# AssafSinger94/dino-tracker

Measured on AMD Instinct MI355X. Metric: query-points*frames/s, higher is better.
Workload: dtype mixed: fp16 ViT operands (one per value), f16 conv operands in Delta-DINO, f16 candidates + f32 deciders in the tracker; f32 accumulate; 1 GPU; 854x480x90 synthetic video (model res 854x476, 67x121 tokens, C=384), 1024 grid queries; 1 video(s) per step over 1 GPU(s); features=vit, mode=single, track_method=mfma, anchor_pairs=92091, correlation_maps_per_video=8380350, rccl_ranks=1, parallelism=video-parallel x1

## Files before the change

dino_tracker_amd/csrc/vit.hip:

```cpp
#include <stdlib.h>
#include "common.h"
#include "vit_attention4.h"
#include "vit_attention6.h"
#include "vit_gemm_common.h"
#include "vit_gemm_tiled.h"
#include "vit_gemm_ws.h"
#include "vit_gemm_wide.h"
#include "vit_split.h"

namespace {

__global__ __launch_bounds__(256) void patch_embed_kernel(const float* __restrict__ frames, const float* __restrict__ Wp,
                                                          const float* __restrict__ bp, const float* __restrict__ pos,
                                                          const float* __restrict__ cls_pos,
                                                          const float* __restrict__ mean_std, float* __restrict__ x,
                                                          int H, int W, int ph, int pw, int D, int patch, int stride,
                                                          int S) {
    const int HW = ph * pw;
    const int K = 3 * patch * patch;
    const int frame = blockIdx.z;
    const int tid = threadIdx.x, lane = tid & 63, w = tid >> 6;
    const int p0 = blockIdx.x * 64 + (w >> 1) * 32;
    const int n0 = blockIdx.y * 64 + (w & 1) * 32;
    const int li = lane & 31, lk = lane >> 5;
// ... 262 lines not shown
VitPlan vit_plan(const dtk_vit_model* m, int ph, int pw, int frames) {
    VitPlan p;
    p.S = ph * pw + 1;
    p.Sp = (p.S + 127) / 128 * 128;
    const int fb = m->frame_batch > 0 ? m->frame_batch : VIT_FRAME_BATCH;
    p.FB = frames < fb ? frames : fb;
    auto al = [](size_t v) { return (v + 255) & ~(size_t)255; };
    size_t off = 0;
    const size_t rows = (size_t)p.FB * p.S;
    p.x = off; off = al(off + rows * m->D * 4);
    p.xn = off; off = al(off + rows * m->D * 2);
    p.q = off; off = al(off + (size_t)p.FB * m->heads * p.Sp * 64 * 2);
    p.k = off; off = al(off + (size_t)p.FB * m->heads * p.Sp * 64 * 2);
    p.vt = off; off = al(off + (size_t)p.FB * m->heads * p.Sp * 64 * 2);
    p.ao = off; off = al(off + rows * m->D * 2);
    p.hid = off; off = al(off + rows * 4 * m->D * 2);
    p.delta = off; off = al(off + rows * m->D * 2);
    p.split = false;
    for (int l = 0; l < m->depth; ++l) p.split |= vit_layer_split(m->layers[l]);
    p.xn_lo = p.q_lo = p.k_lo = p.vt_lo = p.ao_lo = p.hid_lo = 0;
    if (p.split) {
        p.xn_lo = off; off = al(off + rows * m->D * 2);
        p.q_lo = off; off = al(off + (size_t)p.FB * m->heads * p.Sp * 64 * 2);
        p.k_lo = off; off = al(off + (size_t)p.FB * m->heads * p.Sp * 64 * 2);
        p.vt_lo = off; off = al(off + (size_t)p.FB * m->heads * p.Sp * 64 * 2);
        p.ao_lo = off; off = al(off + rows * m->D * 2);
        p.hid_lo = off; off = al(off + rows * 4 * m->D * 2);
    }
    p.total = off;
    return p;
}

template <typename T>
int attention_launch(const T* q, const T* k, const T* vt, T* o, int S, int Sp, int heads, int D, int FH, bool v4, hipStream_t st) {
    int QB;
    if (v4) {
        const unsigned grid = attn::attention_grid(FH, S, 256, &QB);
        DTK_LAUNCH("vit_attention", (attn::attention4_kernel<T, 0>), dim3(grid), dim3(256), 0, st, q, k, vt, o, S, Sp, heads, D,
                   FH, QB);
    } else {
        const unsigned grid = attn::attention_grid(FH, S, 128 * attn::A6_NQ, &QB);
        DTK_LAUNCH("vit_attention", (attn::attention6_kernel<T, 0>), dim3(grid), dim3(256), 0, st, q, k, vt, o, S, Sp, heads, D,
                   FH, QB);
    }
    return DTK_OK;
}

template <typename T>
__global__ __launch_bounds__(256) void range_scan_kernel(const T* __restrict__ p, long long n8, int* __restrict__ flag, int bit) {
    typedef typename Vec<T>::t8 T8;
    bool bad = false;
    for (long long i = (long long)blockIdx.x * 256 + threadIdx.x; i < n8; i += (long long)gridDim.x * 256) {
        const T8 v = reinterpret_cast<const T8*>(p)[i];
#pragma unroll
        for (int e = 0; e < 8; ++e) bad |= !(fabsf((float)v[e]) < 65504.f);
    }
    if (__any(bad) && (threadIdx.x & 63) == 0) atomicOr(flag, bit);
}

struct GemmPath {
    bool tiled;
    bool ws;
    bool wide;
    bool ws_v1;
    bool wide_v1;
    bool fc2_ln;
};
inline GemmPath gemm_path(int D, int f) {
    const bool tiled = (f & DTK_VIT_TILED_GEMMS) != 0, ws = !tiled && D == WS_K, wide_v1 = (f & DTK_VIT_GEMM_WIDE_V1) != 0;
    static_assert(WS_K == WD_N, "fc2 of the weight-stationary width is gemm_wide_delta_kernel's shape");
    return {tiled, ws, !tiled && D % W2_N == 0, (f & DTK_VIT_GEMM_WS_V1) != 0, wide_v1, ws && !wide_v1 && !(f & DTK_VIT_NO_LN_FUSION)};
}
inline GemmPath gemm_path(const dtk_vit_model* m) { return gemm_path(m->D, m->flags); }

template <typename T, int EPI>
int launch_gemm(const char* name, const GemmPath& path, const T* A, const T* W, long long rows, int N, int K, const GemmEpi<T>& e,
                hipStream_t st) {
    if constexpr (EPI != EPI_F32) {
        const bool ws_fits = EPI != EPI_QKV || e.S >= WS_ROWS || rows <= e.S;
        if (path.ws && K == WS_K && ws_fits) {
            const auto gr = gemm_ws_grid(N, rows);
            if (path.ws_v1)
                DTK_LAUNCH(name, (gemm_ws_kernel<T, EPI, 0>), gr.first, dim3(256), 0, st, A, W, rows, N, e, gr.second);
            else
                DTK_LAUNCH(name, (gemm_ws_kernel<T, EPI>), gr.first, dim3(256), 0, st, A, W, rows, N, e, gr.second);
            return DTK_OK;
        }
        if (path.ws && EPI == EPI_DELTA) {
            const dim3 grid(dtk_cdiv(rows, WD_M));
            if (path.wide_v1)
                DTK_LAUNCH(name, (gemm_wide_delta_kernel<T, false>), grid, dim3(512), 0, st, A, W, rows, K, e);
            else if (e.ln_out)
                DTK_LAUNCH(name, (gemm_wide_delta_kernel<T, true, true>), grid, dim3(512), 0, st, A, W, rows, K, e);
            else
                DTK_LAUNCH(name, (gemm_wide_delta_kernel<T, true>), grid, dim3(512), 0, st, A, W, rows, K, e);
            return DTK_OK;
        }
        if (path.wide) {
            const dim3 grid(gemm_wide_grid(N, rows));
            if (path.wide_v1)
                DTK_LAUNCH(name, (gemm_wide_kernel<T, EPI, false>), grid, dim3(512), 0, st, A, W, rows, N, K, e);
            else
                DTK_LAUNCH(name, (gemm_wide_kernel<T, EPI, true>), grid, dim3(512), 0, st, A, W, rows, N, K, e);
            return DTK_OK;
        }
    }
    DTK_LAUNCH(name, (gemm_tiled_kernel<T, EPI>), dim3(gemm_grid(N, rows)), dim3(256), 0, st, A, W, rows, N, K, e);
    return DTK_OK;
}

template <typename T, int SEPI>
int launch_gemm_split(const char* name, const GemmPath& path, const T* Ah, const T* Al, const T* Wh, const T* Wl, long long rows,
                      int N, int K, const SplitEpi<T>& se, hipStream_t st) {
    if (!path.tiled && N % SD_N == 0) {
        const dim3 grid(gemm_split_dma_grid(N, rows));
        if (path.wide_v1)
            DTK_LAUNCH(name, (gemm_split_dma_kernel<T, SEPI, false>), grid, dim3(512), 0, st, Ah, Al, Wh, Wl, rows, N, K, se);
        else
            DTK_LAUNCH(name, (gemm_split_dma_kernel<T, SEPI, true>), grid, dim3(512), 0, st, Ah, Al, Wh, Wl, rows, N, K, se);
        return DTK_OK;
    }
    DTK_LAUNCH(name, (gemm_split_kernel<T, SEPI>), dim3(gemm_split_grid(N, rows)), dim3(256), 0, st, Ah, Al, Wh, Wl, rows, N, K, se);
    return DTK_OK;
}

template <typename T>
int vit_run(const dtk_vit_model* m, const float* frames, int nframes, int video_h, int video_w, float* tokens_out,
            float* feat_out, float* qkv_out, unsigned char* ws, const VitPlan& p, int ph, int pw, hipStream_t st) {
    const int HW = ph * pw, D = m->D;
    float* x = reinterpret_cast<float*>(ws + p.x);
    auto at = [&](size_t off) { return reinterpret_cast<T*>(ws + off); };
    T *xn = at(p.xn), *q = at(p.q), *k = at(p.k), *vt = at(p.vt), *ao = at(p.ao), *hid = at(p.hid), *delta = at(p.delta);
    T *xn_lo = at(p.xn_lo), *q_lo = at(p.q_lo), *k_lo = at(p.k_lo), *vt_lo = at(p.vt_lo), *ao_lo = at(p.ao_lo), *hid_lo = at(p.hid_lo);
    int* ovf = m->overflow;
    const bool scan_all = ovf && (m->flags & DTK_VIT_CHECK_RANGE);
    int* const epi_ovf = IsF16<T>::value ? ovf : nullptr;
    const int S = p.S, Sp = p.Sp;
    {
        const long long n16 = (long long)((p.ao - p.q) / 16);
        DTK_LAUNCH("vit_zero", zero_kernel, dim3(dtk_cdiv(n16, 256)), dim3(256), 0, st, reinterpret_cast<uint4*>(q), n16);
        if (p.split) {
            const long long m16 = (long long)((p.ao_lo - p.q_lo) / 16);
            DTK_LAUNCH("vit_zero", zero_kernel, dim3(dtk_cdiv(m16, 256)), dim3(256), 0, st, reinterpret_cast<uint4*>(q_lo), m16);
        }
    }
    for (int f0 = 0; f0 < nframes; f0 += p.FB) {
        const int nf = (nframes - f0) < p.FB ? (nframes - f0) : p.FB;
        const long long rows = (long long)nf * S;
        auto scan_range = [&](const T* t, long long n, int bit) -> int {
            const int blocks = (int)(dtk_cdiv(n / 8, 256) < 1024 ? dtk_cdiv(n / 8, 256) : 1024);
            DTK_LAUNCH("vit_range_scan", range_scan_kernel<T>, dim3(blocks), dim3(256), 0, st, t, n / 8, ovf, bit);
            return DTK_OK;
        };
        const bool pe_fits = (size_t)nf * video_h * video_w * 16 <= p.delta - p.hid &&
                             (size_t)D * PE_K * 4 <= p.total - p.delta;
        if (m->patch == PE_P && m->stride == PE_S && pe_fits) {
            h4v* fh = reinterpret_cast<h4v*>(hid);
            h4v* fl = fh + (size_t)nf * video_h * video_w;
            half_t* wh = reinterpret_cast<half_t*>(delta);
            half_t* wl = wh + (size_t)D * PE_K;
            const long long npix = (long long)nf * video_h * video_w;
            DTK_LAUNCH("vit_frame_split", frame_split4_kernel, dim3(dtk_cdiv(npix, 256)), dim3(256), 0, st,
                       frames + (size_t)f0 * 3 * video_h * video_w, m->mean_std, fh, fl, video_h, video_w, npix);
            DTK_LAUNCH("vit_frame_split", pack_patch_split_kernel, dim3(dtk_cdiv((long long)D * PE_K, 256)), dim3(256), 0, st,
                       m->patch_w, D, wh, wl);
            const int groups_x = dtk_cdiv(pw, PE_TOK);
            const int units = groups_x * ph * nf, slabs = dtk_cdiv(D, PE_NF);
            DTK_LAUNCH("vit_patch_embed", patch_embed_split_kernel, dim3(8 * dtk_cdiv(units, 8) * slabs), dim3(256), 0, st, fh,
                       fl, wh, wl, m->patch_b, m->pos, m->cls_pos, x, video_h, video_w, ph, pw, D, S, groups_x, units, slabs);
        } else {
            DTK_LAUNCH("vit_patch_embed", patch_embed_kernel, dim3(dtk_cdiv(HW, 64), dtk_cdiv(D, 64), nf), dim3(256), 0, st,
                       frames + (size_t)f0 * 3 * video_h * video_w, m->patch_w, m->patch_b, m->pos, m->cls_pos, m->mean_std,
                       x, video_h, video_w, ph, pw, D, m->patch, m->stride, S);
        }
        const GemmPath path = gemm_path(m);
        const int dbg_ns = DTK_DBG(dtk_dev_flags() >> 16, 0x7f);
        bool pending = false;
        bool ln1_done = false;
        auto tap = [&](int l, bool with_delta) -> int {
            if (!m->tap_out || !((m->tap_mask >> l) & 1)) return DTK_OK;
            const long long t4 = rows * (D / 4);
            DTK_LAUNCH("vit_tap", tap_kernel<T>, dim3(dtk_cdiv(t4, 256)), dim3(256), 0, st, x, with_delta ? (const T*)delta : (const T*)nullptr,
                       m->tap_out + (size_t)f0 * S * D, m->tap_scale, t4);
            return DTK_OK;
        };
        for (int l = 0; l < m->depth; ++l) {
            const dtk_vit_layer& L = m->layers[l];
            const T* qkv_w = reinterpret_cast<const T*>(L.qkv_w);
            const T* proj_w = reinterpret_cast<const T*>(L.proj_w);
            const T* fc1_w = reinterpret_cast<const T*>(L.fc1_w);
            const T* fc2_w = reinterpret_cast<const T*>(L.fc2_w);
            if (vit_layer_split(L)) {
                const T* qkv_wl = reinterpret_cast<const T*>(L.qkv_w_lo);
                const T* proj_wl = reinterpret_cast<const T*>(L.proj_w_lo);
                const T* fc1_wl = reinterpret_cast<const T*>(L.fc1_w_lo);
                const T* fc2_wl = reinterpret_cast<const T*>(L.fc2_w_lo);
                const float inv_ws = 1.f / (L.w_scale > 0.f ? L.w_scale : 1.f);
                DTK_LAUNCH("vit_layernorm_split", layernorm_split_kernel<T>, dim3(dtk_cdiv(rows, 4)), dim3(256), 0, st, x,
                           pending ? (const T*)delta : (const T*)nullptr, L.ln1_w, L.ln1_b, xn, xn_lo, rows, D, m->ln_eps, ovf);
                pending = false;
                SplitEpi<T> se{};
                if (qkv_out && l == m->depth - 1) {
                    se.bias = L.qkv_b; se.inv_wscale = inv_ws; se.out_f32 = qkv_out + (size_t)f0 * S * 3 * D;
                    if (launch_gemm_split<T, SEPI_F32>("vit_gemm_qkv_facet", path, xn, xn_lo, qkv_w, qkv_wl, rows, 3 * D, D, se, st)) return DTK_E_HIP;
                    se = SplitEpi<T>{};
                }
                se.bias = L.qkv_b; se.inv_wscale = inv_ws; se.q_hi = q; se.q_lo = q_lo; se.k_hi = k; se.k_lo = k_lo; se.vt_hi = vt;
                se.vt_lo = vt_lo; se.S = S; se.Sp = Sp; se.heads = m->heads; se.D = D; se.qscale = 0.125f * 1.4426950408889634f;
                se.ovf = epi_ovf;
                if (launch_gemm_split<T, SEPI_QKV>("vit_gemm_qkv_split", path, xn, xn_lo, qkv_w, qkv_wl, rows, 3 * D, D, se, st)) return DTK_E_HIP;
                const int nqb = dtk_cdiv(Sp, 128);
                DTK_LAUNCH("vit_attention_split", attention_split_kernel<T>, dim3((unsigned)(nf * m->heads * nqb)), dim3(256), 0, st,
                           (const T*)q, (const T*)q_lo, (const T*)k, (const T*)k_lo, (const T*)vt, (const T*)vt_lo, ao, ao_lo, S, Sp,
                           m->heads, nqb);
                se = SplitEpi<T>{};
                se.bias = L.proj_b; se.inv_wscale = inv_ws; se.x = x; se.gamma = L.ls1;
                if (launch_gemm_split<T, SEPI_RESID>("vit_gemm_proj_split", path, ao, ao_lo, proj_w, proj_wl, rows, D, D, se, st)) return DTK_E_HIP;
                DTK_LAUNCH("vit_layernorm_split", layernorm_split_kernel<T>, dim3(dtk_cdiv(rows, 4)), dim3(256), 0, st, x,
                           (const T*)nullptr, L.ln2_w, L.ln2_b, xn, xn_lo, rows, D, m->ln_eps, ovf);
                se = SplitEpi<T>{};
                se.bias = L.fc1_b; se.inv_wscale = inv_ws; se.out_hi = hid; se.out_lo = hid_lo; se.ovf = epi_ovf;
                if (launch_gemm_split<T, SEPI_GELU>("vit_gemm_fc1_split", path, xn, xn_lo, fc1_w, fc1_wl, rows, 4 * D, D, se, st)) return DTK_E_HIP;
                se = SplitEpi<T>{};
                se.bias = L.fc2_b; se.inv_wscale = inv_ws; se.x = x; se.gamma = L.ls2;
                if (launch_gemm_split<T, SEPI_RESID>("vit_gemm_fc2_split", path, hid, hid_lo, fc2_w, fc2_wl, rows, D, 4 * D, se, st)) return DTK_E_HIP;
                if (tap(l, false)) return DTK_E_HIP;
                continue;
            }
            GemmEpi<T> e{};
            if (!ln1_done)
                DTK_LAUNCH("vit_layernorm", layernorm_kernel<T>, dim3(dtk_cdiv(rows, 4)), dim3(256), 0, st, x,
                           pending ? (const T*)delta : (const T*)nullptr, L.ln1_w, L.ln1_b, xn, rows, D, m->ln_eps, ovf);
            ln1_done = false;
            pending = true;
            if (qkv_out && l == m->depth - 1) {
                e.bias = L.qkv_b; e.out_f32 = qkv_out + (size_t)f0 * S * 3 * D;
                if (launch_gemm<T, EPI_F32>("vit_gemm_qkv_facet", path, xn, qkv_w, rows, 3 * D, D, e, st)) return DTK_E_HIP;
                e = GemmEpi<T>{};
            }
            e.bias = L.qkv_b; e.q = q; e.k = k; e.vt = vt; e.S = S; e.Sp = Sp; e.heads = m->heads; e.D = D;
            e.qscale = 0.125f * 1.4426950408889634f; e.no_store = dbg_ns; e.ovf = epi_ovf;
            if (launch_gemm<T, EPI_QKV>("vit_gemm_qkv", path, xn, qkv_w, rows, 3 * D, D, e, st)) return DTK_E_HIP;
            if (scan_all && scan_range(q, (long long)(p.ao - p.q) / 2, 2)) return DTK_E_HIP;
            if (attention_launch(q, k, vt, ao, S, Sp, m->heads, D, nf * m->heads, (m->flags & DTK_VIT_ATTENTION_V4) != 0, st)) return DTK_E_HIP;
            e = GemmEpi<T>{};
            e.bias = L.proj_b; e.delta = delta; e.gamma = L.ls1; e.no_store = dbg_ns;
            if (launch_gemm<T, EPI_DELTA>("vit_gemm_proj", path, ao, proj_w, rows, D, D, e, st)) return DTK_E_HIP;
            DTK_LAUNCH("vit_layernorm", layernorm_kernel<T>, dim3(dtk_cdiv(rows, 4)), dim3(256), 0, st, x, (const T*)delta,
                       L.ln2_w, L.ln2_b, xn, rows, D, m->ln_eps, ovf);
            e = GemmEpi<T>{};
            e.bias = L.fc1_b; e.out = hid; e.no_store = dbg_ns; e.ovf = epi_ovf;
            if (launch_gemm<T, EPI_GELU>("vit_gemm_fc1", path, xn, fc1_w, rows, 4 * D, D, e, st)) return DTK_E_HIP;
            if (scan_all && scan_range(hid, rows * 4 * D, 4)) return DTK_E_HIP;
            e = GemmEpi<T>{};
            e.bias = L.fc2_b; e.delta = delta; e.gamma = L.ls2; e.no_store = dbg_ns;
            if (path.fc2_ln && l + 1 < m->depth && !vit_layer_split(m->layers[l + 1])) {
                const dtk_vit_layer& Ln = m->layers[l + 1];
                e.ln_x = x; e.ln_w = Ln.ln1_w; e.ln_b = Ln.ln1_b; e.ln_out = xn; e.ln_eps = m->ln_eps; e.ln_ovf = ovf;
                pending = false;
// ... 205 lines not shown
```

dino_tracker_amd/csrc/vit_gemm_common.h:

```cpp
#pragma once
#include "common.h"

namespace {

typedef float f2 __attribute__((ext_vector_type(2)));
typedef float f4 __attribute__((ext_vector_type(4)));
typedef float f16v __attribute__((ext_vector_type(16)));
typedef _Float16 half_t;
typedef _Float16 h8 __attribute__((ext_vector_type(8)));
typedef _Float16 h4v __attribute__((ext_vector_type(4)));
typedef __bf16 bf8 __attribute__((ext_vector_type(8)));

template <typename T> struct Vec {
    typedef T t8 __attribute__((ext_vector_type(8)));
    typedef T t4 __attribute__((ext_vector_type(4)));
};
template <typename T> struct IsF16 { static constexpr bool value = false; };
template <> struct IsF16<_Float16> { static constexpr bool value = true; };
__device__ __forceinline__ f4 mfma16(h8 a, h8 b, f4 c) { return __builtin_amdgcn_mfma_f32_16x16x32_f16(a, b, c, 0, 0, 0); }
__device__ __forceinline__ f4 mfma16(bf8 a, bf8 b, f4 c) { return __builtin_amdgcn_mfma_f32_16x16x32_bf16(a, b, c, 0, 0, 0); }
__device__ __forceinline__ f16v mfma32(h8 a, h8 b, f16v c) { return __builtin_amdgcn_mfma_f32_32x32x16_f16(a, b, c, 0, 0, 0); }
__device__ __forceinline__ f16v mfma32(bf8 a, bf8 b, f16v c) { return __builtin_amdgcn_mfma_f32_32x32x16_bf16(a, b, c, 0, 0, 0); }
template <typename T> __device__ __forceinline__ void operand_mode() {
    if (IsF16<T>::value) dtk_fp16_saturate_mode();
}

constexpr int GM = 128, GN = 128, GK = 32;
enum { EPI_QKV = 0, EPI_GELU = 1, EPI_DELTA = 2, EPI_F32 = 3 };

template <typename T>
struct GemmEpi {
    const float* bias;
    T* q;
    T* k;
    T* vt;
    int S, Sp, heads, D;
    float qscale;
    T* out;
    int no_store;
    T* delta;
    const float* gamma;
    float* out_f32;
    int* ovf;
    float* ln_x;
    const float *ln_w, *ln_b;
    T* ln_out;
    float ln_eps;
    int* ln_ovf;
};

__device__ __forceinline__ float amax2(float m, float a, float b) { return fmaxf(fmaxf(m, fabsf(a)), fabsf(b)); }
template <typename T, int EPI>
__device__ __forceinline__ void amax_report(float amax, int* ovf) {
    if (IsF16<T>::value && (EPI == EPI_QKV || EPI == EPI_GELU) && ovf) {
        if (__any(amax >= 65488.f) && (threadIdx.x & 63) == 0) atomicOr(ovf, EPI == EPI_QKV ? 2 : 4);
    }
}

__device__ __forceinline__ int gswz_f(int row) { return (0x1230 >> (((row >> 2) & 3) * 4)) & 3; }
__device__ __forceinline__ int gswz(int row, int piece) { return row * 4 + (piece ^ gswz_f(row)); }
__device__ __forceinline__ uint4 staged16(const unsigned char* sp) {
    const uint2 lo = *reinterpret_cast<const uint2*>(sp), hi = *reinterpret_cast<const uint2*>(sp + 8);
    return make_uint4(lo.x, lo.y, hi.x, hi.y);
}

template <typename T, int EPI>
__device__ __forceinline__ void gemm_store_tile(const f4& a, long long mb, int n, float bias, long long M, int N,
                                                const GemmEpi<T>& e, float& amax) {
    if (IsF16<T>::value && (EPI == EPI_QKV || EPI == EPI_GELU)) {
        const float sc = (EPI == EPI_QKV && n < e.D) ? e.qscale : 1.f;
        if (EPI == EPI_GELU) amax = fmaxf(fmaxf(fmaxf(amax, a[0] + bias), fmaxf(a[1] + bias, a[2] + bias)), a[3] + bias);
        else amax = amax2(amax2(amax, (a[0] + bias) * sc, (a[1] + bias) * sc), (a[2] + bias) * sc, (a[3] + bias) * sc);
    }
    if (EPI == EPI_QKV) {
        const int which = n / e.D, rem = n - which * e.D;
        const int head = rem >> 6, dh = rem & 63;
        const int frame = (int)(mb / e.S);
        (void)frame;
        if (which == 2) {
#pragma unroll
            for (int r = 0; r < 4; ++r) {
                const long long m = mb + r;
                if (m < M) {
                    const int f = (int)(m / e.S), s = (int)(m - (long long)f * e.S);
                    e.vt[(((size_t)f * e.heads + head) * 64 + dh) * e.Sp + s] = (T)(a[r] + bias);
                }
            }
        } else {
            T* dst = which == 0 ? e.q : e.k;
            const float sc = which == 0 ? e.qscale : 1.f;
#pragma unroll
            for (int r = 0; r < 4; ++r) {
                const long long m = mb + r;
                if (m < M) {
                    const int f = (int)(m / e.S), s = (int)(m - (long long)f * e.S);
                    dst[(((size_t)f * e.heads + head) * e.Sp + s) * 64 + dh] = (T)((a[r] + bias) * sc);
                }
            }
// ... 100 lines not shown
```

dino_tracker_amd/csrc/vit_gemm_ws.h:

```cpp
#pragma once
#include <utility>
#include "vit_gemm_common.h"

namespace {

constexpr int WS_KS = 24, WS_K = 16 * WS_KS, WS_ROWS = 32, WS_COLS = 256;
constexpr int WS_TILE_BYTES = WS_ROWS * WS_K * 2;
constexpr int WS_LQ = WS_KS / 4;
constexpr int WS_PITCH = 144;
constexpr int WS_UNIT_BYTES = WS_ROWS * WS_PITCH;

template <typename T, int EPI, int V2M = 3>
__global__ __launch_bounds__(256) void gemm_ws_kernel(const T* __restrict__ A, const T* __restrict__ Wt,
                                                      long long M, int N, GemmEpi<T> e, int tiles_per_chunk) {
    typedef typename Vec<T>::t8 T8;
    typedef typename Vec<T>::t4 T4;
    (void)sizeof(T8); (void)sizeof(T4);
    constexpr bool V2 = (V2M & 1) != 0;
    constexpr bool V2D = (V2M & 2) != 0;
    operand_mode<T>();
    __shared__ __attribute__((aligned(1024))) unsigned char toks[3][WS_TILE_BYTES];
    __shared__ __attribute__((aligned(16))) unsigned char stage[4][2][WS_UNIT_BYTES];
    __shared__ __attribute__((aligned(16))) float s_bias[4][64], s_gamma[4][64];
    const int tid = threadIdx.x, lane = tid & 63;
    const int w = __builtin_amdgcn_readfirstlane(tid >> 6);
    const int j = lane & 31, h = lane >> 5;
    const int n0 = blockIdx.x * WS_COLS + w * 64;
    const long long total_tiles = (M + WS_ROWS - 1) / WS_ROWS;
    const long long tile0 = (long long)blockIdx.y * tiles_per_chunk;
    if (tile0 >= total_tiles) return;
    const int NT = (int)((total_tiles - tile0) < tiles_per_chunk ? (total_tiles - tile0) : tiles_per_chunk);
    const int nl = (j & 3) + 4 * (j >> 3) + 16 * ((j >> 2) & 1);
    T8 wf[2][WS_KS];
#pragma unroll
    for (int t = 0; t < 2; ++t) {
        const int row = min(n0 + t * 32 + nl, N - 1);
        const T* wp = Wt + (size_t)row * WS_K + h * 8;
#pragma unroll
        for (int ks = 0; ks < WS_KS; ++ks) {
            if (V2) asm volatile("global_load_dwordx4 %0, %1, off" : "=a"(wf[t][ks]) : "v"(wp + ks * 16) : "memory");
            else wf[t][ks] = *reinterpret_cast<const T8*>(wp + ks * 16);
        }
    }
    if (V2) {
        asm volatile("s_waitcnt vmcnt(0)" ::: "memory");
#pragma unroll
        for (int t = 0; t < 2; ++t)
#pragma unroll
            for (int ks = 0; ks < WS_KS; ++ks) asm volatile("" : "+a"(wf[t][ks]));
    }
    {
        const int n = min(n0 + lane, N - 1);
        s_bias[w][lane] = e.bias ? e.bias[n] : 0.f;
        s_gamma[w][lane] = (EPI == EPI_DELTA) ? e.gamma[n] : 1.f;
    }
    const int which = (EPI == EPI_QKV) ? min(n0, N - 1) / e.D : 0;
    const int head = (EPI == EPI_QKV) ? (min(n0, N - 1) - which * e.D) >> 6 : 0;
    const float qsc = (EPI == EPI_QKV && which == 0) ? e.qscale : 1.f;
    long long m_ep = tile0 * WS_ROWS + j;
    int f_ep = 0, s_ep = 0;
    if (EPI == EPI_QKV) { f_ep = (int)(m_ep / e.S); s_ep = (int)(m_ep - (long long)f_ep * e.S); }
    const unsigned lds_base = (unsigned)(size_t)&toks[0][0];
    const int l_tt = lane & 3, l_pp = lane >> 2;
    const dtk_u4 srd = dtk_make_srd(A + tile0 * WS_ROWS * WS_K);
    unsigned a_voff[2], a_voff_last[2];
    const int last_rows = (int)(M - (total_tiles - 1) * WS_ROWS);
#pragma unroll
    for (int gg = 0; gg < 2; ++gg) {
        const int g = 2 * w + gg;
        a_voff[gg] = (unsigned)(((4 * g + l_tt) * WS_K + ((l_pp - g) & 15) * 8) * 2);
        a_voff_last[gg] = (unsigned)((min(4 * g + l_tt, last_rows - 1) * WS_K + ((l_pp - g) & 15) * 8) * 2);
    }
    const unsigned a_dst = __builtin_amdgcn_readfirstlane(lds_base + (2 * w) * 3 * 1024);
    auto issue = [&](int n, int buf) {
        if (V2D) {
            const unsigned toff = __builtin_amdgcn_readfirstlane((unsigned)n * (unsigned)WS_TILE_BYTES);
            const unsigned dst = __builtin_amdgcn_readfirstlane(a_dst + (unsigned)buf * (unsigned)WS_TILE_BYTES);
            const bool last = tile0 + n == total_tiles - 1;
            const unsigned v0 = last ? a_voff_last[0] : a_voff[0], v1 = last ? a_voff_last[1] : a_voff[1];
            dtk_buffer_lds16<0>(srd, toff, v0, dst);
            dtk_buffer_lds16<1024>(srd, toff + 256u, v0, dst);
            dtk_buffer_lds16<2048>(srd, toff + 512u, v0, dst);
            dtk_buffer_lds16<3072>(srd, toff, v1, dst);
            dtk_buffer_lds16<4096>(srd, toff + 256u, v1, dst);
            dtk_buffer_lds16<5120>(srd, toff + 512u, v1, dst);
            return;
        }
#pragma unroll
        for (int gg = 0; gg < 2; ++gg) {
            const int g = 2 * w + gg;
            const long long m = min((tile0 + n) * WS_ROWS + 4 * g + l_tt, M - 1);
            const T* gp = A + m * WS_K + ((l_pp - g) & 15) * 8;
#pragma unroll
            for (int c = 0; c < 3; ++c)
                dtk_glds16(gp + c * 128, __builtin_amdgcn_readfirstlane(lds_base + buf * WS_TILE_BYTES + (g * 3 + c) * 1024));
        }
    };
    unsigned frag_off[8];
#pragma unroll
    for (int k8 = 0; k8 < 8; ++k8)
        frag_off[k8] = (unsigned)((j >> 2) * 3 * 1024 + ((((2 * k8 + h + (j >> 2)) & 15) * 4 + (j & 3)) * 16));
    float amax = 0.f;
    auto epi8 = [&](const f16v (&acc)[2], int t, int hv) {
        const int fl = 32 * t + 16 * h + 8 * hv;
        const int nb = n0 + fl;
        const float4 b0 = *reinterpret_cast<const float4*>(&s_bias[w][fl]), b1 = *reinterpret_cast<const float4*>(&s_bias[w][fl + 4]);
        float v[8];
#pragma unroll
        for (int r = 0; r < 8; ++r) v[r] = acc[t][8 * hv + r];
        v[0] += b0.x; v[1] += b0.y; v[2] += b0.z; v[3] += b0.w;
        v[4] += b1.x; v[5] += b1.y; v[6] += b1.z; v[7] += b1.w;
        const bool ok = m_ep < M && nb < N && !DTK_DBG(e.no_store, 3);
        if (IsF16<T>::value && (EPI == EPI_QKV || EPI == EPI_GELU)) {
#pragma unroll
            for (int r = 0; r < 8; r += 2) {
                if (EPI == EPI_GELU) amax = fmaxf(fmaxf(amax, v[r]), v[r + 1]);
                else amax = amax2(amax, v[r] * qsc, v[r + 1] * qsc);
            }
        }
        if (EPI == EPI_GELU) {
            T8 o;
#pragma unroll
            for (int r = 0; r < 8; r += 2) {
                const f2 g = gelu2(f2{v[r], v[r + 1]});
                o[r] = (T)g[0];
                o[r + 1] = (T)g[1];
            }
            if (ok) *reinterpret_cast<T8*>(e.out + m_ep * N + nb) = o;
        } else if (EPI == EPI_DELTA) {
            const float4 g0 = *reinterpret_cast<const float4*>(&s_gamma[w][fl]), g1 = *reinterpret_cast<const float4*>(&s_gamma[w][fl + 4]);
            T8 o = {(T)(v[0] * g0.x), (T)(v[1] * g0.y), (T)(v[2] * g0.z), (T)(v[3] * g0.w),
                     (T)(v[4] * g1.x), (T)(v[5] * g1.y), (T)(v[6] * g1.z), (T)(v[7] * g1.w)};
            *reinterpret_cast<T8*>(&stage[w][0][0] + j * WS_PITCH + fl * 2) = o;
        } else {
            const int dh = fl;
            if (which == 2) {
                if (ok) {
                    T* vp = e.vt + (((size_t)f_ep * e.heads + head) * 64 + dh) * e.Sp + s_ep;
#pragma unroll
                    for (int r = 0; r < 8; ++r) vp[(size_t)r * e.Sp] = (T)v[r];
                }
            } else {
                T8 o;
#pragma unroll
                for (int r = 0; r < 8; ++r) o[r] = (T)(v[r] * qsc);
                *reinterpret_cast<T8*>(&stage[w][0][0] + j * WS_PITCH + fl * 2) = o;
            }
        }
    };
    long long mt_fl = tile0 * WS_ROWS;
    int f0_fl = 0, s0_fl = 0;
    if (EPI == EPI_QKV) { f0_fl = (int)(mt_fl / e.S); s0_fl = (int)(mt_fl - (long long)f0_fl * e.S); }
    auto flush = [&]() {
        if (EPI != EPI_GELU && n0 < N && !DTK_DBG(e.no_store, 3) && !(EPI == EPI_QKV && which == 2)) {
#pragma unroll
            for (int u = 0; u < 1; ++u) {
#pragma unroll
                for (int p = 0; p < 4; ++p) {
                    const int row = 8 * p + (lane >> 3), piece = lane & 7;
                    const uint4 val = *reinterpret_cast<const uint4*>(&stage[w][u][0] + row * WS_PITCH + piece * 16);
                    if (mt_fl + row < M) {
                        if (EPI == EPI_DELTA) {
                            *reinterpret_cast<uint4*>(e.delta + (mt_fl + row) * N + n0 + piece * 8) = val;
                        } else {
                            int f = f0_fl, sp = s0_fl + row;
                            if (sp >= e.S) { sp -= e.S; ++f; }
                            T* dst = which == 0 ? e.q : e.k;
                            *reinterpret_cast<uint4*>(dst + (((size_t)f * e.heads + head) * e.Sp + sp) * 64 + piece * 8) = val;
                        }
                    }
                }
            }
        }
        mt_fl += WS_ROWS;
        if (EPI == EPI_QKV) {
            s0_fl += WS_ROWS;
            if (s0_fl >= e.S) { s0_fl -= e.S; ++f0_fl; }
        }
    };
    auto advance = [&]() {
        m_ep += WS_ROWS;
        if (EPI == EPI_QKV) {
            s_ep += WS_ROWS;
            if (s_ep >= e.S) { s_ep -= e.S; ++f_ep; }
        }
    };
    auto step = [&](int buf, f16v (&accN)[2], const f16v (&accP)[2], bool have_prev, bool have_flush) {
        if (!V2) {
#pragma unroll
            for (int t = 0; t < 2; ++t)
#pragma unroll
                for (int r = 0; r < 16; ++r) accN[t][r] = 0.f;
        }
        const unsigned char* base = &toks[0][0] + buf * WS_TILE_BYTES;
        const f16v zero16 = {0.f, 0.f, 0.f, 0.f, 0.f, 0.f, 0.f, 0.f, 0.f, 0.f, 0.f, 0.f, 0.f, 0.f, 0.f, 0.f};
        T8 b[3];
        b[0] = *reinterpret_cast<const T8*>(base + frag_off[0]);
        b[1] = *reinterpret_cast<const T8*>(base + frag_off[1]);
#pragma unroll
        for (int ks = 0; ks < WS_KS; ++ks) {
            if (ks + 2 < WS_KS)
                b[(ks + 2) % 3] = *reinterpret_cast<const T8*>(base + frag_off[(ks + 2) & 7] + ((ks + 2) >> 3) * 1024);
#pragma unroll
            for (int t = 0; t < 2; ++t) {
                if (V2) accN[t] = mfma32(wf[t][ks], b[ks % 3], ks == 0 ? zero16 : accN[t]);
                else accN[t] = mfma32(wf[t][ks], b[ks % 3], accN[t]);
            }
            if (have_flush && ks == 0) flush();
            if (have_prev && ks % 6 == 2) epi8(accP, (ks / 6) >> 1, (ks / 6) & 1);
        }
        if (have_prev) advance();
    };
    f16v accA[2], accB[2];
    issue(0, 0);
    issue(min(1, NT - 1), 1);
    dtk_vm_wait<WS_LQ>();
    __syncthreads();
    int n = 0, b0 = 0;
    for (; n + 1 < NT; n += 2) {
        const int b1 = b0 == 2 ? 0 : b0 + 1, b2 = b1 == 2 ? 0 : b1 + 1;
        issue(min(n + 2, NT - 1), b2);
        step(b0, accA, accB, n > 0, n > 1);
        dtk_vm_wait<WS_LQ>();
        __syncthreads();
        issue(min(n + 3, NT - 1), b0);
        step(b1, accB, accA, true, n > 0);
        dtk_vm_wait<WS_LQ>();
        __syncthreads();
        b0 = b2;
    }
    if (n < NT) {
        step(b0, accA, accB, n > 0, n > 1);
        if (n > 0) flush();
#pragma unroll
        for (int u = 0; u < 4; ++u) epi8(accA, u >> 1, u & 1);
    } else {
        if (n > 1) flush();
#pragma unroll
        for (int u = 0; u < 4; ++u) epi8(accB, u >> 1, u & 1);
    }
    flush();
    amax_report<T, EPI>(amax, e.ovf);
    dtk_vm_wait<0>();
}

inline std::pair<dim3, int> gemm_ws_grid(int N, long long rows) {
    const int colwg = dtk_cdiv(N, WS_COLS);
    const int chunks = 256 / colwg > 0 ? 256 / colwg : 1;
    const long long tiles = dtk_cdiv(rows, WS_ROWS);
    const int tpc = (int)dtk_cdiv(tiles, chunks);
    return std::make_pair(dim3(colwg, (unsigned)dtk_cdiv(tiles, tpc)), tpc);
}

}
```

Before: 515,600 query-points*frames/s.

## Interleave GEMM epilogue slots with MFMA steps in weight-stationary kernel

Adds a hand-scheduled variant of the weight-stationary GEMM in which the previous tile's epilogue (bias, GELU polynomial, scaling, staging and stores) is cut into per-MFMA slots and placed between the MFMAs of the next tile using scheduling barriers. Bias and gamma are held in registers instead of LDS. The variant becomes the default when N is a multiple of 64, and the old path stays as a fallback. The aim is to hide epilogue ALU and store latency behind matrix-core work, at the cost of more register pressure and a rigid instruction order. Debug flags for skipping stores and arithmetic are also added.

```diff
diff --git a/dino_tracker_amd/csrc/vit.hip b/dino_tracker_amd/csrc/vit.hip
--- a/dino_tracker_amd/csrc/vit.hip
+++ b/dino_tracker_amd/csrc/vit.hip
@@ -368,6 +368,8 @@
             const auto gr = gemm_ws_grid(N, rows);
             if (path.ws_v1)
                 DTK_LAUNCH(name, (gemm_ws_kernel<T, EPI, 0>), gr.first, dim3(256), 0, st, A, W, rows, N, e, gr.second);
+            else if (N % 64 != 0 || DTK_DBG(e.no_store, 128))
+                DTK_LAUNCH(name, (gemm_ws_kernel<T, EPI, 3, false>), gr.first, dim3(256), 0, st, A, W, rows, N, e, gr.second);
             else
                 DTK_LAUNCH(name, (gemm_ws_kernel<T, EPI>), gr.first, dim3(256), 0, st, A, W, rows, N, e, gr.second);
             return DTK_OK;
@@ -460,7 +462,7 @@
                        x, video_h, video_w, ph, pw, D, m->patch, m->stride, S);
         }
         const GemmPath path = gemm_path(m);
-        const int dbg_ns = DTK_DBG(dtk_dev_flags() >> 16, 0x7f);
+        const int dbg_ns = DTK_DBG(dtk_dev_flags() >> 16, 0xff);
         bool pending = false;
         bool ln1_done = false;
         auto tap = [&](int l, bool with_delta) -> int {
diff --git a/dino_tracker_amd/csrc/vit_gemm_common.h b/dino_tracker_amd/csrc/vit_gemm_common.h
--- a/dino_tracker_amd/csrc/vit_gemm_common.h
+++ b/dino_tracker_amd/csrc/vit_gemm_common.h
@@ -14,6 +14,7 @@
 template <typename T> struct Vec {
     typedef T t8 __attribute__((ext_vector_type(8)));
     typedef T t4 __attribute__((ext_vector_type(4)));
+    typedef T t2 __attribute__((ext_vector_type(2)));
 };
 template <typename T> struct IsF16 { static constexpr bool value = false; };
 template <> struct IsF16<_Float16> { static constexpr bool value = true; };
diff --git a/dino_tracker_amd/csrc/vit_gemm_ws.h b/dino_tracker_amd/csrc/vit_gemm_ws.h
--- a/dino_tracker_amd/csrc/vit_gemm_ws.h
+++ b/dino_tracker_amd/csrc/vit_gemm_ws.h
@@ -1,4 +1,5 @@
 #pragma once
+#include <type_traits>
 #include <utility>
 #include "vit_gemm_common.h"
 
@@ -10,7 +11,12 @@
 constexpr int WS_PITCH = 144;
 constexpr int WS_UNIT_BYTES = WS_ROWS * WS_PITCH;
 
-template <typename T, int EPI, int V2M = 3>
+template <class F, int... I>
+__device__ __forceinline__ void ws_for_each(F&& f, std::integer_sequence<int, I...>) { (f(std::integral_constant<int, I>{}), ...); }
+template <int N, class F>
+__device__ __forceinline__ void ws_for_each(F&& f) { ws_for_each(f, std::make_integer_sequence<int, N>{}); }
+
+template <typename T, int EPI, int V2M = 3, bool HC = (V2M == 3)>
 __global__ __launch_bounds__(256) void gemm_ws_kernel(const T* __restrict__ A, const T* __restrict__ Wt,
                                                       long long M, int N, GemmEpi<T> e, int tiles_per_chunk) {
     typedef typename Vec<T>::t8 T8;
@@ -18,6 +24,7 @@
     (void)sizeof(T8); (void)sizeof(T4);
     constexpr bool V2 = (V2M & 1) != 0;
     constexpr bool V2D = (V2M & 2) != 0;
+    static_assert(!HC || V2M == 3, "the hand-cut step is built on the AGPR weights and the descriptor LDS-DMA");
     operand_mode<T>();
     __shared__ __attribute__((aligned(1024))) unsigned char toks[3][WS_TILE_BYTES];
     __shared__ __attribute__((aligned(16))) unsigned char stage[4][2][WS_UNIT_BYTES];
@@ -49,7 +56,7 @@
 #pragma unroll
             for (int ks = 0; ks < WS_KS; ++ks) asm volatile("" : "+a"(wf[t][ks]));
     }
-    {
+    if constexpr (!HC) {
         const int n = min(n0 + lane, N - 1);
         s_bias[w][lane] = e.bias ? e.bias[n] : 0.f;
         s_gamma[w][lane] = (EPI == EPI_DELTA) ? e.gamma[n] : 1.f;
@@ -101,6 +108,258 @@
     for (int k8 = 0; k8 < 8; ++k8)
         frag_off[k8] = (unsigned)((j >> 2) * 3 * 1024 + ((((2 * k8 + h + (j >> 2)) & 15) * 4 + (j & 3)) * 16));
     float amax = 0.f;
+    unsigned dbg_sink = 0;
+    auto dbg_fold = [&](const auto& val) {
+        unsigned b[sizeof(val) / 4];
+        __builtin_memcpy(b, &val, sizeof(val));
+#pragma unroll
+        for (unsigned i = 0; i < sizeof(val) / 4; ++i) dbg_sink |= b[i];
+    };
+    if constexpr (HC) {
+        typedef std::integral_constant<bool, true> Yes;
+        typedef std::integral_constant<bool, false> No;
+        if (n0 >= N) {
+            issue(0, 0);
+            issue(min(1, NT - 1), 1);
+            dtk_vm_wait<WS_LQ>();
+            __syncthreads();
+            int b0 = 0;
+            for (int n = 0; n + 1 < NT; n += 2) {
+                const int b1 = b0 == 2 ? 0 : b0 + 1, b2 = b1 == 2 ? 0 : b1 + 1;
+                issue(min(n + 2, NT - 1), b2);
+                dtk_vm_wait<WS_LQ>();
+                __syncthreads();
+                issue(min(n + 3, NT - 1), b0);
+                dtk_vm_wait<WS_LQ>();
+                __syncthreads();
+                b0 = b2;
+            }
+            dtk_vm_wait<0>();
+            return;
+        }
+        float bia[2][16], gam[2][16];
+#pragma unroll
+        for (int t = 0; t < 2; ++t)
+#pragma unroll
+            for (int r = 0; r < 16; ++r) {
+                const int nf = n0 + 32 * t + 16 * h + r;
+                bia[t][r] = e.bias ? e.bias[nf] : 0.f;
+                gam[t][r] = (EPI == EPI_DELTA) ? e.gamma[nf] : 1.f;
+            }
+        const bool dbg_nost = DTK_DBG(e.no_store, 3) || DTK_DBG(e.no_store, 32);
+        const bool dbg_noar = DTK_DBG(e.no_store, 64);
+        auto run = [&](auto vt_tag) {
+            constexpr bool VT = decltype(vt_tag)::value;
+            constexpr bool STG = EPI != EPI_GELU && !VT;
+            const long long mt0 = tile0 * WS_ROWS;
+            T* op = nullptr;
+            T* up = nullptr;
+            int s0 = 0;
+            unsigned cross = 0;
+            if constexpr (EPI == EPI_GELU) op = e.out + (mt0 + j) * N + n0 + 16 * h;
+            if constexpr (EPI == EPI_DELTA) up = e.delta + mt0 * N + n0;
+            if constexpr (EPI == EPI_QKV) {
+                const int f0 = (int)(mt0 / e.S);
+                s0 = (int)(mt0 - (long long)f0 * e.S);
+                if (VT) {
+                    up = e.vt + (((size_t)f0 * e.heads + head) * 64) * e.Sp + s0;
+                    cross = (unsigned)(e.heads * 64 * e.Sp - e.S);
+                } else {
+                    up = (which == 0 ? e.q : e.k) + (((size_t)f0 * e.heads + head) * e.Sp + s0) * 64;
+                    cross = (unsigned)((e.heads * e.Sp - e.S) * 64);
+                }
+            }
+            const size_t out_step = (size_t)WS_ROWS * N;
+            unsigned char* const sw = &stage[w][0][0] + j * WS_PITCH + 32 * h;
+            const unsigned char* const sr = &stage[w][0][0] + (lane >> 3) * WS_PITCH + (lane & 7) * 16;
+            auto next_tile = [&]() {
+                if constexpr (EPI == EPI_GELU) op += out_step;
+                if constexpr (EPI == EPI_DELTA) up += out_step;
+                if constexpr (EPI == EPI_QKV) {
+                    s0 += WS_ROWS;
+                    up += VT ? WS_ROWS : WS_ROWS * 64;
+                    if (s0 >= e.S) { s0 -= e.S; up += cross; }
+                }
+            };
+            auto st16 = [&](T* p, unsigned off, dtk_u4 val, bool ok) {
+                if (!dbg_nost) { if (ok) *reinterpret_cast<dtk_u4*>(p + off) = val; }
+                else dbg_fold(val);
+            };
+            float v[8];
+            f2 sx[4], uu[4], pp[4];
+            T8 o;
+            dtk_u4 fv[4];
+            unsigned voff = 0;
+            constexpr float GC[9] = {1.112979639e-10f, -1.065557687e-08f, 4.510875158e-07f, -1.125288873e-05f, 1.868377149e-04f,
+                                     -2.217123518e-03f, 1.963194646e-02f, -1.326889843e-01f, 7.978046536e-01f};
+            auto flush_reads = [&]() {
+                ws_for_each<4>([&](auto p_tag) {
+                    constexpr int p = decltype(p_tag)::value;
+                    fv[p] = *reinterpret_cast<const dtk_u4*>(sr + 8 * p * WS_PITCH);
+                });
+            };
+            auto flush_store = [&](auto pred_tag, auto p_tag, int valid) {
+                constexpr int p = decltype(p_tag)::value;
+                const int row = 8 * p + (lane >> 3);
+                const bool ok = decltype(pred_tag)::value ? row < valid : true;
+                if constexpr (EPI == EPI_DELTA) st16(up, (unsigned)(row * N + (lane & 7) * 8), fv[p], ok);
+                else st16(up, (unsigned)(row * 64 + (lane & 7) * 8) + (s0 + row >= e.S ? cross : 0u), fv[p], ok);
+            };
+            auto slot = [&](auto pred_tag, auto fl_tag, const f16v (&acc)[2], auto s_tag, int valid) {
+                constexpr bool PRED = decltype(pred_tag)::value, FL = decltype(fl_tag)::value;
+                constexpr int s = decltype(s_tag)::value;
+                const bool ok = PRED ? j < valid : true;
+                if constexpr (EPI == EPI_GELU) {
+                    constexpr int u = s / 12, ph = s % 12, t = u >> 1, hv = u & 1;
+                    if (ph < 2) {
+#pragma unroll
+                        for (int r = 4 * ph; r < 4 * ph + 4; ++r) v[r] = acc[t][8 * hv + r] + bia[t][8 * hv + r];
+                        if (IsF16<T>::value) {
+#pragma unroll
+                            for (int r = 4 * ph; r < 4 * ph + 4; r += 2) amax = fmaxf(fmaxf(amax, v[r]), v[r + 1]);
+                        }
+                    }
+                    if (dbg_noar) {
+                        if (ph == 9) {
+#pragma unroll
+                            for (int r = 0; r < 8; ++r) o[r] = (T)v[r];
+                        }
+                    } else if (ph == 2) {
+                        const f2 c = {4.25f, 4.25f};
+#pragma unroll
+                        for (int q = 0; q < 4; ++q) sx[q] = __builtin_elementwise_min(__builtin_elementwise_max(f2{v[2 * q], v[2 * q + 1]}, -c), c);
+#pragma unroll
+                        for (int q = 0; q < 4; ++q) uu[q] = sx[q] * sx[q];
+                    } else if (ph >= 3 && ph <= 6) {
+#pragma unroll
+                        for (int l = 2 * (ph - 3); l < 2 * (ph - 3) + 2; ++l)
+#pragma unroll
+                            for (int q = 0; q < 4; ++q)
+                                pp[q] = __builtin_elementwise_fma(l == 0 ? f2{GC[0], GC[0]} : pp[q], uu[q], f2{GC[l + 1], GC[l + 1]});
+                    } else if (ph == 7) {
+                        const f2 one = {1.f, 1.f};
+#pragma unroll
+                        for (int q = 0; q < 4; ++q) pp[q] = __builtin_elementwise_min(__builtin_elementwise_max(sx[q] * pp[q], -one), one);
+                    } else if (ph == 8) {
+#pragma unroll
+                        for (int q = 0; q < 4; ++q) {
+                            const f2 hx = f2{v[2 * q], v[2 * q + 1]} * f2{0.5f, 0.5f};
+                            uu[q] = __builtin_elementwise_fma(hx, pp[q], hx);
+                        }
+                    } else if (ph == 9) {
+#pragma unroll
+                        for (int q = 0; q < 4; ++q) { o[2 * q] = (T)uu[q][0]; o[2 * q + 1] = (T)uu[q][1]; }
+                    }
+                    if (ph == 10) {
+                        st16(op, (unsigned)(32 * t + 8 * hv), __builtin_bit_cast(dtk_u4, o), ok);
+                    }
+                } else if constexpr (STG) {
+                    if constexpr (FL && s == 0) flush_reads();
+                    if constexpr (FL && s >= 1 && s <= 4) flush_store(No{}, std::integral_constant<int, s - 1>{}, WS_ROWS);
+                    constexpr int u = s / 12, ph = s % 12, t = u >> 1, hv = u & 1;
+                    if (ph & 1) {
+                        if (ph < 9) {
+                            constexpr int r0 = (ph - 1) & 7, r1 = ph & 7;
+                            const float v0 = acc[t][8 * hv + r0] + bia[t][8 * hv + r0], v1 = acc[t][8 * hv + r1] + bia[t][8 * hv + r1];
+                            if (EPI == EPI_QKV && IsF16<T>::value && !dbg_noar) amax = amax2(amax, v0 * qsc, v1 * qsc);
+                            if (dbg_noar) { o[r0] = (T)v0; o[r1] = (T)v1; }
+                            else if (EPI == EPI_DELTA) { o[r0] = (T)(v0 * gam[t][8 * hv + r0]); o[r1] = (T)(v1 * gam[t][8 * hv + r1]); }
+                            else { o[r0] = (T)(v0 * qsc); o[r1] = (T)(v1 * qsc); }
+                        } else if (ph == 9) {
+                            *reinterpret_cast<T8*>(sw + 64 * t + 16 * hv) = o;
+                        }
+                    }
+                } else {
+                    if (s == 0) voff = (unsigned)(16 * h * e.Sp + j) + (s0 + j >= e.S ? cross : 0u);
+                    if (s < 32) {
+                        constexpr int u = (s & 31) / 8, r = s % 8, t = u >> 1, hv = u & 1;
+                        v[r] = acc[t][8 * hv + r] + bia[t][8 * hv + r];
+                        if (IsF16<T>::value && (r & 1) && !dbg_noar) amax = amax2(amax, v[r - 1] * qsc, v[r] * qsc);
+                        const T val = (T)v[r];
+                        T* const p = up + (size_t)(32 * t + 8 * hv + r) * e.Sp;
+                        if (!dbg_nost) { if (ok) p[voff] = val; }
+                        else dbg_fold(typename Vec<T>::t2{val, val});
+                    }
+                }
+            };
+            auto tail_epi = [&](const f16v (&acc)[2], int valid) {
+                ws_for_each<2 * WS_KS>([&](auto s_tag) { slot(Yes{}, No{}, acc, s_tag, valid); });
+                if (!STG) next_tile();
+            };
+            auto tail_flush = [&](int valid) {
+                if constexpr (STG) {
+                    flush_reads();
+                    ws_for_each<4>([&](auto p_tag) { flush_store(Yes{}, p_tag, valid); });
+                    next_tile();
+                }
+            };
+            auto step = [&](auto prev_tag, auto fl_tag, int buf, f16v (&accN)[2], const f16v (&accP)[2]) {
+                constexpr bool PREV = decltype(prev_tag)::value, FL = decltype(fl_tag)::value;
+                const unsigned char* base = &toks[0][0] + buf * WS_TILE_BYTES;
+                const f16v zero16 = {0.f, 0.f, 0.f, 0.f, 0.f, 0.f, 0.f, 0.f, 0.f, 0.f, 0.f, 0.f, 0.f, 0.f, 0.f, 0.f};
+                T8 b[3];
+                b[0] = *reinterpret_cast<const T8*>(base + frag_off[0]);
+                b[1] = *reinterpret_cast<const T8*>(base + frag_off[1]);
+                ws_for_each<2 * WS_KS>([&](auto s_tag) {
+                    constexpr int ks = decltype(s_tag)::value / 2, t = decltype(s_tag)::value % 2;
+                    if constexpr (t == 0 && ks + 2 < WS_KS)
+                        b[(ks + 2) % 3] = *reinterpret_cast<const T8*>(base + frag_off[(ks + 2) & 7] + ((ks + 2) >> 3) * 1024);
+                    accN[t] = mfma32(wf[t][ks], b[ks % 3], ks == 0 ? zero16 : accN[t]);
+                    if constexpr (PREV) {
+                        __builtin_amdgcn_sched_barrier(0);
+                        slot(No{}, fl_tag, accP, s_tag, WS_ROWS);
+                        __builtin_amdgcn_sched_barrier(0);
+                    }
+                });
+                if (STG ? FL : PREV) next_tile();
+            };
+            f16v accA[2], accB[2];
+            issue(0, 0);
+            issue(min(1, NT - 1), 1);
+            dtk_vm_wait<WS_LQ>();
+            __syncthreads();
+            int n = 0, b0 = 0;
+            auto pair = [&](auto first_tag) {
+                constexpr bool FIRST = decltype(first_tag)::value;
+                const int b1 = b0 == 2 ? 0 : b0 + 1, b2 = b1 == 2 ? 0 : b1 + 1;
+                issue(min(n + 2, NT - 1), b2);
+                if (FIRST) step(No{}, No{}, b0, accA, accB);
+                else step(Yes{}, Yes{}, b0, accA, accB);
+                dtk_vm_wait<WS_LQ>();
+                __syncthreads();
+                issue(min(n + 3, NT - 1), b0);
+                if (FIRST) step(Yes{}, No{}, b1, accB, accA);
+                else step(Yes{}, Yes{}, b1, accB, accA);
+                dtk_vm_wait<WS_LQ>();
+                __syncthreads();
+                b0 = b2;
+                n += 2;
+            };
+            if (NT >= 2) pair(Yes{});
+            while (n + 1 < NT) pair(No{});
+            const long long left = M - (tile0 + NT - 1) * WS_ROWS;
+            const int valid = left < WS_ROWS ? (int)left : WS_ROWS;
+            const bool odd = n < NT;
+            if (odd) {
+                if (n > 0) step(Yes{}, Yes{}, b0, accA, accB);
+                else step(No{}, No{}, b0, accA, accB);
+            }
+            if (NT > 1) tail_flush(WS_ROWS);
+            const f16v accL[2] = {odd ? accA[0] : accB[0], odd ? accA[1] : accB[1]};
+            tail_epi(accL, valid);
+            tail_flush(valid);
+        };
+        if constexpr (EPI == EPI_QKV) {
+            if (which == 2) run(Yes{});
+            else run(No{});
+        } else {
+            run(No{});
+        }
+        if (DTK_DBG(e.no_store, 32) && dbg_sink == 0x9e3779b9u) amax = 65504.f;
+        amax_report<T, EPI>(amax, e.ovf);
+        dtk_vm_wait<0>();
+        return;
+    }
     auto epi8 = [&](const f16v (&acc)[2], int t, int hv) {
         const int fl = 32 * t + 16 * h + 8 * hv;
         const int nb = n0 + fl;
@@ -115,18 +374,19 @@
 #pragma unroll
             for (int r = 0; r < 8; r += 2) {
                 if (EPI == EPI_GELU) amax = fmaxf(fmaxf(amax, v[r]), v[r + 1]);
-                else amax = amax2(amax, v[r] * qsc, v[r + 1] * qsc);
+                else if (!DTK_DBG(e.no_store, 64)) amax = amax2(amax, v[r] * qsc, v[r + 1] * qsc);
             }
         }
         if (EPI == EPI_GELU) {
             T8 o;
 #pragma unroll
             for (int r = 0; r < 8; r += 2) {
-                const f2 g = gelu2(f2{v[r], v[r + 1]});
+                const f2 g = DTK_DBG(e.no_store, 64) ? f2{v[r], v[r + 1]} : gelu2(f2{v[r], v[r + 1]});
                 o[r] = (T)g[0];
                 o[r + 1] = (T)g[1];
             }
-            if (ok) *reinterpret_cast<T8*>(e.out + m_ep * N + nb) = o;
+            if (DTK_DBG(e.no_store, 32)) dbg_fold(o);
+            else if (ok) *reinterpret_cast<T8*>(e.out + m_ep * N + nb) = o;
         } else if (EPI == EPI_DELTA) {
             const float4 g0 = *reinterpret_cast<const float4*>(&s_gamma[w][fl]), g1 = *reinterpret_cast<const float4*>(&s_gamma[w][fl + 4]);
             T8 o = {(T)(v[0] * g0.x), (T)(v[1] * g0.y), (T)(v[2] * g0.z), (T)(v[3] * g0.w),
@@ -135,7 +395,10 @@
         } else {
             const int dh = fl;
             if (which == 2) {
-                if (ok) {
+                if (DTK_DBG(e.no_store, 32)) {
+#pragma unroll
+                    for (int r = 0; r < 8; r += 2) dbg_fold(typename Vec<T>::t2{(T)v[r], (T)v[r + 1]});
+                } else if (ok) {
                     T* vp = e.vt + (((size_t)f_ep * e.heads + head) * 64 + dh) * e.Sp + s_ep;
 #pragma unroll
                     for (int r = 0; r < 8; ++r) vp[(size_t)r * e.Sp] = (T)v[r];
@@ -143,7 +406,7 @@
             } else {
                 T8 o;
 #pragma unroll
-                for (int r = 0; r < 8; ++r) o[r] = (T)(v[r] * qsc);
+                for (int r = 0; r < 8; ++r) o[r] = DTK_DBG(e.no_store, 64) ? (T)v[r] : (T)(v[r] * qsc);
                 *reinterpret_cast<T8*>(&stage[w][0][0] + j * WS_PITCH + fl * 2) = o;
             }
         }
@@ -159,7 +422,8 @@
                 for (int p = 0; p < 4; ++p) {
                     const int row = 8 * p + (lane >> 3), piece = lane & 7;
                     const uint4 val = *reinterpret_cast<const uint4*>(&stage[w][u][0] + row * WS_PITCH + piece * 16);
-                    if (mt_fl + row < M) {
+                    if (DTK_DBG(e.no_store, 32)) dbg_fold(val);
+                    else if (mt_fl + row < M) {
                         if (EPI == EPI_DELTA) {
                             *reinterpret_cast<uint4*>(e.delta + (mt_fl + row) * N + n0 + piece * 8) = val;
                         } else {
@@ -240,6 +504,7 @@
         for (int u = 0; u < 4; ++u) epi8(accB, u >> 1, u & 1);
     }
     flush();
+    if (DTK_DBG(e.no_store, 32) && dbg_sink == 0x9e3779b9u) amax = 65504.f;
     amax_report<T, EPI>(amax, e.ovf);
     dtk_vm_wait<0>();
 }
```

Result: faster. 522,700 query-points*frames/s, median of 6 (+1.4%).
